# mmdagent/distantspeechrecognition-mirror

Hardware: AMD Instinct MI355X
Metric: decoded_audio_hours_per_sec (higher is better)
Workload: dtype f32

## Files before the change

### distantspeechrecognition-mirror_amd/csrc/k_viterbi.hip

```cpp
#include "common.h"
#include "wfst_graph.h"
#include "lattice.h"
#include "lexicon.h"
#include "wordtrace.h"
#include <algorithm>
#include <cmath>
#include <type_traits>

namespace dsr {

struct Tok { int32_t node; float ac; float lm; uint32_t bp; };
struct TokA { float ac; float lm; uint32_t bp; uint32_t xs; };
struct TokB { int32_t node; int32_t cnt; };
struct XRecD { int32_t dist; float cost; uint32_t meta; float eps1; int32_t dst; int32_t p2; int32_t dstXoff; int32_t dstCnt; };
struct Side { double ttl; float ac; float lm; int32_t rec; uint32_t prevBp; int32_t c; uint32_t next; };
struct CandA { double ttl; float ac; float lm; };
struct CandB { int32_t dst; int32_t next; int32_t rec; uint32_t prevBp; };
struct Bp { uint32_t prev; uint32_t rec; };

static constexpr uint32_t kNone = 0xFFFFFFFFu;
static constexpr uint32_t kEndBit = 0x80000000u;
static constexpr int kThreads = 1024;
static constexpr int kWaves = kThreads / 64;
static constexpr int kFastK = 8;
static constexpr int kB = 2;
static constexpr int kFastC = 24576;
static constexpr int kFastE = 8190;
static constexpr int kP1 = 16;
static constexpr int kW = 4;
static constexpr int kSideLds = 496;

struct GraphDev {
  int nNodes, initial;
  const int* xoff; const XRec* xrec; const XRecD* xrecD; const int* xarc; const int* xpathOff;
  const int* eoff; const ERec* erec; const int* path; const float* pathCost;
  const float* arcCost; const uint32_t* arcOut; const uint32_t* arcIn;
  const int* nodeFinal; const float* nodeCost;
};

struct SegState { int n, status, maxActive, pad; long arenaOff, chunkEnd, arenaUsed; double thresh; long long stat[3]; };

struct DecDev {
  double beam, lmScale, lmPenalty, silPenalty; uint32_t silenceX; int noPen;
  int segFrames, segCount, segQueues, segDrop; long poolCap, poolChunk;    unsigned long long* poolNext; SegState* segState; int* segDone; TokA* saveA; TokB* saveB;
  int maxTok, maxCand; long arenaCap;
  TokA* tokA; TokB* tokB; TokA* ctok; Side* side; int fastOK; int* tokOff; int* tokCnt; int* owner; int* rank; int* chead; CandA* cA; CandB* cB; unsigned* first; unsigned* tags; Bp* arena;
  int* queue; long long* prof;
  int dumpOn; long dumpCap; long* dumpFrameOff; int* dumpNode; float* dumpAc; float* dumpLm; int* dumpArc; long* dumpCount;
  int latOn; long latCap; uint4* lat; double* latTtl; long* latFrameOff; int* arenaLat; int4* latFinal; int* latInfo;
  int topN; TokA* tokA3; TokB* tokB3;
};

struct VitArgs {
  GraphDev G; DecDev D;
  const float* scores; const int* nframesArr; int U, Tmax, nDist;
  dsr_decode_result* res; int* arcsOut; unsigned* wordsOut; int maxPath, useLdsRow, hashN, regionB, cntCap;
};
typedef const __attribute__((address_space(4))) VitArgs* KP;

__device__ __forceinline__ unsigned ld_u32(const unsigned* p) { return __hip_atomic_load(p, __ATOMIC_RELAXED, __HIP_MEMORY_SCOPE_AGENT); }
__device__ __forceinline__ int ld_i32(const int* p) { return __hip_atomic_load(p, __ATOMIC_RELAXED, __HIP_MEMORY_SCOPE_AGENT); }
__device__ __forceinline__ void st_u32(unsigned* p, unsigned v) { __hip_atomic_store(p, v, __ATOMIC_RELAXED, __HIP_MEMORY_SCOPE_AGENT); }
__device__ __forceinline__ void st_i32(int* p, int v) { __hip_atomic_store(p, v, __ATOMIC_RELAXED, __HIP_MEMORY_SCOPE_AGENT); }
__device__ __forceinline__ void st_u64_dev(void* p, unsigned long long v) { __hip_atomic_store(reinterpret_cast<unsigned long long*>(p), v, __ATOMIC_RELAXED, __HIP_MEMORY_SCOPE_AGENT); }
__device__ __forceinline__ unsigned long long ld_u64_dev(const void* p) { return __hip_atomic_load(reinterpret_cast<const unsigned long long*>(p), __ATOMIC_RELAXED, __HIP_MEMORY_SCOPE_AGENT); }

__device__ __forceinline__ int wave_incl_scan(int v, int )
{
  v += __builtin_amdgcn_update_dpp(0, v, 0x111, 0xF, 0xF, true);
  v += __builtin_amdgcn_update_dpp(0, v, 0x112, 0xF, 0xF, true);
  v += __builtin_amdgcn_update_dpp(0, v, 0x114, 0xF, 0xF, true);
  v += __builtin_amdgcn_update_dpp(0, v, 0x118, 0xF, 0xF, true);
  v += __builtin_amdgcn_update_dpp(0, v, 0x142, 0xA, 0xF, false);
  v += __builtin_amdgcn_update_dpp(0, v, 0x143, 0xC, 0xF, false);
  return v;
}
__device__ __forceinline__ float wave_max_f_uni(float v)
{
#define DSR_DPP_F(ctrl, rm) { const float o = __int_as_float(__builtin_amdgcn_update_dpp(__float_as_int(v), __float_as_int(v), ctrl, rm, 0xF, false)); v = fmaxf(v, o); }
  DSR_DPP_F(0x111, 0xF) DSR_DPP_F(0x112, 0xF) DSR_DPP_F(0x114, 0xF) DSR_DPP_F(0x118, 0xF) DSR_DPP_F(0x142, 0xA) DSR_DPP_F(0x143, 0xC)
#undef DSR_DPP_F
  return __int_as_float(__builtin_amdgcn_readlane(__float_as_int(v), 63));
}
__device__ __forceinline__ double wave_min_d_uni(double v)
{
#define DSR_DPP_D(ctrl, rm) { const int lo = __double2loint(v), hi = __double2hiint(v); \
    const double o = __hiloint2double(__builtin_amdgcn_update_dpp(hi, hi, ctrl, rm, 0xF, false), __builtin_amdgcn_update_dpp(lo, lo, ctrl, rm, 0xF, false)); v = (o < v) ? o : v; }
  DSR_DPP_D(0x111, 0xF) DSR_DPP_D(0x112, 0xF) DSR_DPP_D(0x114, 0xF) DSR_DPP_D(0x118, 0xF) DSR_DPP_D(0x142, 0xA) DSR_DPP_D(0x143, 0xC)
#undef DSR_DPP_D
  return __hiloint2double(__builtin_amdgcn_readlane(__double2hiint(v), 63), __builtin_amdgcn_readlane(__double2loint(v), 63));
}
__device__ __forceinline__ double wave_min_d(double v)
{
#pragma unroll
  for (int d = 32; d >= 1; d >>= 1) { const double o = __shfl_xor(v, d, 64); v = (o < v) ? o : v; }
  return v;
}
__device__ __forceinline__ unsigned long long wave_min_u64(unsigned long long v)
{
// ... 27 lines not shown
{
  if (idx < sideLds) {
    const lds_side_t* p = (const lds_side_t*) sideL + idx;
    const unsigned long long a = *reinterpret_cast<const volatile __attribute__((address_space(3))) unsigned long long*>(&p->ac);
    rec = *reinterpret_cast<const volatile __attribute__((address_space(3))) int*>(&p->rec);
    ac = __uint_as_float((unsigned) (a & 0xFFFFFFFFull)); lm = __uint_as_float((unsigned) (a >> 32));
    DSR_NO_MERGE();
  } else {
    const Side* p = side + idx;
    const unsigned long long a = *reinterpret_cast<const volatile unsigned long long*>(&p->ac); rec = *reinterpret_cast<const volatile int*>(&p->rec);
    ac = __uint_as_float((unsigned) (a & 0xFFFFFFFFull)); lm = __uint_as_float((unsigned) (a >> 32));
  }
}
__device__ __forceinline__ void side_link(const Side* sideL, const Side* side, int sideLds, int idx, int& c, double& ttl, unsigned& next)
{
  if (idx < sideLds) { const lds_side_t* p = (const lds_side_t*) sideL + idx; c = p->c; ttl = p->ttl; next = p->next; DSR_NO_MERGE(); }
  else { const Side* p = side + idx; c = p->c; ttl = p->ttl; next = p->next; }
}
__device__ __forceinline__ float side_score(const Side* sideL, const Side* side, int sideLds, int idx)
{
  float r;
  if (idx < sideLds) { const lds_side_t* p = (const lds_side_t*) sideL + idx; r = __fadd_rn(p->ac, p->lm); DSR_NO_MERGE(); }
  else { const Side* p = side + idx; r = __fadd_rn(p->ac, p->lm); }
  return r;
}
template <class T> __device__ __forceinline__ const T* at32(const void* base, uint32_t byteOff) { return reinterpret_cast<const T*>(reinterpret_cast<const char*>(base) + byteOff); }
template <class T> __device__ __forceinline__ T* at32w(void* base, uint32_t byteOff) { return reinterpret_cast<T*>(reinterpret_cast<char*>(base) + byteOff); }
__device__ __forceinline__ int uni(int v) { return __builtin_amdgcn_readfirstlane(v); }
__device__ __forceinline__ double uni(double v) { return __hiloint2double(__builtin_amdgcn_readfirstlane(__double2hiint(v)), __builtin_amdgcn_readfirstlane(__double2loint(v))); }
__device__ __forceinline__ unsigned f2ord(float f) { const unsigned u = __float_as_uint(f); return (u & 0x80000000u) ? ~u : (u | 0x80000000u); }

template <int MODES>
__global__ __launch_bounds__(kThreads) void k_viterbi(const VitArgs argsInKernarg)
{
  (void) argsInKernarg;
  constexpr bool PROF = (MODES & 1) != 0, EXTRA = (MODES & 2) != 0;
  const KP KA = (KP) __builtin_amdgcn_kernarg_segment_ptr();
  KP ka = KA;
#define RELOAD() do { ka = KA; asm volatile("" : "+s"(ka)); } while (0)
  RELOAD();
  extern __shared__ __attribute__((aligned(16))) unsigned char smem[];
  float* srow = reinterpret_cast<float*>(smem);
  const int useLdsRow = ka->useLdsRow, nDist = ka->nDist, hashN = ka->hashN, regionB = ka->regionB, cntCap = ka->cntCap;
  unsigned* hkey = reinterpret_cast<unsigned*>(srow + (useLdsRow ? ((nDist + 3) & ~3) : 4));
  unsigned* hfirst = hkey + hashN;
  Side* sideL = reinterpret_cast<Side*>(hfirst + hashN);
  unsigned short* cntL = reinterpret_cast<unsigned short*>(reinterpret_cast<unsigned char*>(hfirst + hashN) + regionB);
  __shared__ int s_waveTot[kWaves];
  __shared__ int s_waveTotE[kWaves];
  __shared__ double s_waveMin[kWaves];
  __shared__ float s_waveMag[kWaves];
  __shared__ unsigned long long s_waveKey[kWaves];
  __shared__ int s_sideN;
  __shared__ int s_tb[2];
  __shared__ unsigned s_bm[kFastC / 32];
  __shared__ unsigned s_gbase[kFastC / 64 + 4];
  __shared__ int s_cnt[(kFastK + 32) * kWaves];
  __shared__ int s_err;
  __shared__ long long s_prof[32]; __shared__ long long s_tlast;
  __shared__ long long s_stat[3];
  __shared__ int s_maxActive; __shared__ unsigned s_tag; __shared__ long long s_latOff;
  if (PROF && threadIdx.x < 32) s_prof[threadIdx.x] = 0;
#define TICK(ix) do { if (PROF && tid == 0) { const long long tn = (long long) wall_clock64(); s_prof[ix] += tn - s_tlast; s_tlast = tn; } } while (0)
  constexpr int nthr = kThreads, nw = kWaves;
  __shared__ int s_u, s_seg, s_help; __shared__ long long s_chunk;

  const int tid = threadIdx.x;
  const int slot = blockIdx.x;
#define TOKA(ix) ((EXTRA && (ix) == 2) ? ka->D.tokA3 + (size_t) slot * ka->D.maxTok : ka->D.tokA + ((size_t) slot * 2 + (size_t) (ix)) * ka->D.maxTok)
#define TOKB(ix) ((EXTRA && (ix) == 2) ? ka->D.tokB3 + (size_t) slot * ka->D.maxTok : ka->D.tokB + ((size_t) slot * 2 + (size_t) (ix)) * ka->D.maxTok)
#define curA TOKA(bufCur)
#define nxtA TOKA(bufNxt)
#define curB TOKB(bufCur)
#define nxtB TOKB(bufNxt)
#define sprA TOKA(bufSpr)
#define sprB TOKB(bufSpr)
#define ctok (ka->D.ctok + (size_t) slot * 8192)
#define side (ka->D.side + (size_t) slot * kFastC)
#define cA (ka->D.cA + (size_t) slot * ka->D.maxCand)
#define cB (ka->D.cB + (size_t) slot * ka->D.maxCand)
  if (tid == 0) s_tag = ka->D.tags[slot];
#define arena (ka->D.arena + (size_t) ((EXTRA && ka->D.latOn) ? u : (ka->D.segFrames > 0 ? 0 : slot)) * ka->D.arenaCap)
#define sc (ka->scores + (size_t) u * ka->Tmax * nDist)
  constexpr int fastCapC = ((kFastK + 32) * nthr < kFastC) ? (kFastK + 32) * nthr : kFastC;
  constexpr int fastCapN = kP1 * 64 * nw;
  const bool fastOK = ka->D.fastOK && hashN >= 8192;
  const int tableC = (hashN >> 1) + (hashN >> 2), eCap = kFastE, sideLds = regionB >> 5;

  const int nq = (EXTRA || ka->D.segFrames <= 0) ? 1 : ka->D.segQueues;
  const int xcd = nq == 8 ? (int) (__builtin_amdgcn_s_getreg((3 << 11) | 20) & 7u) : 0;
  if (tid == 0) s_help = (nq == 8 && ((ka->D.segDrop >> xcd) & 1)) ? 1 : 0;
  for (;;) {
    __syncthreads();
    if (tid == 0) {
      const int segS0 = EXTRA ? 0 : ka->D.segFrames; int help = s_help, uu = -1, sg = 0;
      for (;;) {
        const int qx = (xcd + help) & (nq - 1), Uq = (ka->U - qx + nq - 1) / nq;
        int it = -1;
        if (help == 0) { it = atomicAdd(ka->D.queue + qx, 1); if (it >= (segS0 > 0 ? ka->D.segCount * Uq : Uq)) it = -1; }
        else {
          int c = ld_i32(ka->D.queue + qx);
          while (c < Uq) { const int prev = atomicCAS(ka->D.queue + qx, c, c + 1); if (prev == c) { it = c; break; } c = prev; }
        }
        if (it >= 0) { uu = segS0 > 0 ? qx + nq * (it % Uq) : it; sg = segS0 > 0 ? it / Uq : 0; break; }
        if (segS0 > 0 && nq == 8 && help < 7) help++; else break;
      }
      if (uu >= 0 && help > 0) { st_i32(&ka->D.segState[uu].status, -2); asm volatile("s_waitcnt vmcnt(0)" ::: "memory"); st_i32(&ka->D.segDone[uu], 0x7FFFFFFF); sg = -1; }
// ... 842 lines not shown
              nxtA[pos] = na; nxtB[pos] = nb; arena[arenaOff + pos] = bp;
              if (EXTRA && ka->D.latOn) ka->D.arenaLat[(size_t) u * ka->D.arenaCap + arenaOff + pos] = (int) (s_latOff + w);
            }
          }
        }
      }
      if (EXTRA && ka->D.latOn) {
        uint4* lat = ka->D.lat + (size_t) u * ka->D.latCap; double* ltt = ka->D.latTtl + (size_t) u * ka->D.latCap;
        const long latOff = (long) s_latOff;
        for (int c = tid; c < C; c += nthr) {
          const CandA a = cA[c]; const CandB b = cB[c];
          lat[latOff + c] = make_uint4(__float_as_uint(a.ac), __float_as_uint(a.lm), (unsigned) b.rec, b.prevBp); ltt[latOff + c] = a.ttl;
        }
        __syncthreads();
        if (tid == 0) { s_latOff = latOff + C; ka->D.latFrameOff[(size_t) u * (ka->Tmax + 3) + fr + 1] = latOff + C; }
      }
      }
      __syncthreads();
      TICK(fast ? 7 : 8);
      RELOAD();
      if (mode == 0) {
        if (dump) {
          long* cnt = ka->D.dumpCount; const long o = cnt[0];
          if (o + numNew <= ka->D.dumpCap) {
            for (int i = tid; i < numNew; i += nthr) {
              const TokA t = ld_tok(&nxtA[i]); ka->D.dumpNode[o + i] = nxtB[i].node; ka->D.dumpAc[o + i] = t.ac; ka->D.dumpLm[o + i] = t.lm;
              ka->D.dumpArc[o + i] = ka->G.xarc[arena[t.bp].rec];
            }
          }
          __syncthreads();
          if (tid == 0) { ka->D.dumpFrameOff[fr] = o; ka->D.dumpFrameOff[fr + 1] = o + numNew; cnt[0] = o + numNew; cnt[1] = fr + 1; }
        }
        if (numStat < 0) numStat = numNew;
        if (numStat == 0 || numNew == 0) { status = DSR_E_CONSISTENCY; break; }
        { const int t = bufCur; bufCur = bufNxt; bufNxt = t; }
        n = numNew; arenaOff += numNew; arenaUsed += numNew;
        if (tid == nthr - 1) { s_stat[0] += numStat; s_stat[1] += Cfr; if (fast) s_stat[2] += 1; if (numStat > s_maxActive) s_maxActive = numStat; }
        thresh = __dadd_rn(topScore, ka->D.beam);
      } else {
        const TokA* lst = numNew > 0 ? nxtA : curA; const int cntL = numNew > 0 ? numNew : n;
        unsigned long long key = ~0ull;
        for (int i = tid; i < cntL; i += nthr) {
          const TokA t = lst[i]; const float s = __fadd_rn(t.ac, t.lm);
          if (s == s) { const unsigned long long k = ((unsigned long long) f2ord(s) << 32) | (unsigned) i; if (k < key) key = k; }
        }
        key = wave_min_u64(key);
        if (lane == 0) s_waveKey[wave] = key;
        if (EXTRA && ka->D.latOn) {
          const TokB* lstB = numNew > 0 ? nxtB : curB; int4* lf = ka->D.latFinal + (size_t) u * ka->D.maxTok;
          for (int i = tid; i < cntL; i += nthr) { const TokA t = ld_tok(&lst[i]); lf[i] = make_int4(lstB[i].node, (int) t.bp, __float_as_int(t.ac), __float_as_int(t.lm)); }
          if (tid == 0) { int* li = ka->D.latInfo + 4 * (size_t) u; li[0] = cntL; li[1] = numNew > 0 ? 1 : 0; li[2] = (int) (arenaOff + (numNew > 0 ? numNew : 0)); li[3] = T; }
        }
        __syncthreads();
        int* hopRec = reinterpret_cast<int*>(cB); const int hopCap = 2 * ka->D.maxCand; int* hopOff = hopRec + hopCap;
        if (tid == 0) {
          dsr_decode_result* const res = ka->res;
          clear_result(&res[u]); dsr_decode_result& r = res[u];
          unsigned long long k = ~0ull; for (int w = 0; w < nw; w++) if (s_waveKey[w] < k) k = s_waveKey[w];
          r.frames = T - 1; r.reachedFinal = numNew > 0 ? 1 : 0; r.finalStatesN = numNew;  r.activeHypos = (long) s_stat[0]; r.placements = (long) s_stat[1] + Cfr; r.registerFrames = (long) s_stat[2]; r.maxActiveSeen = s_maxActive; r.status = DSR_OK;
          int nH = 0;
          if (k != ~0ull) {
            const TokA bt = ld_tok(&lst[(unsigned) (k & 0xFFFFFFFFu)]);
            r.ac = bt.ac; r.lm = bt.lm; r.score = __dadd_rn((double) bt.ac, (double) bt.lm);
            for (uint32_t bq = bt.bp; bq != kNone && nH < hopCap; ) {
              uint2 e; if (segS > 0) { const unsigned long long v = ld_u64_dev(&arena[bq]); e.x = (unsigned) v; e.y = (unsigned) (v >> 32); } else e = *reinterpret_cast<const uint2*>(&arena[bq]);
              hopRec[nH++] = (int) e.y; bq = e.x;
            }
          } else r.status = DSR_E_CONSISTENCY;
          s_tb[0] = nH; s_tb[1] = 0;
        }
        __syncthreads();
        const int nH = s_tb[0];
        auto block_excl = [&](const int v, int& total) -> int {
          const int incl = wave_incl_scan(v, lane);
          if (lane == 63) s_waveTot[wave] = incl;
          __syncthreads();
          int base = 0, tot = 0;
          for (int w = 0; w < nw; w++) { const int q = s_waveTot[w]; if (w < wave) base += q; tot += q; }
          __syncthreads();
          total = tot; return base + incl - v;
        };
        int nA = 0;
        for (int b0 = 0; b0 < nH; b0 += nthr) {
          const int i = b0 + tid; int len = 0;
          if (i < nH) { const uint32_t rc = (uint32_t) hopRec[i]; len = (rc & kEndBit) ? ka->G.erec[rc & ~kEndBit].pathLen : (int) (ka->G.xrec[rc].meta & 0xFFFFu) + 1; }
          int total; const int ex = block_excl(len, total);
          if (i < nH) hopOff[i] = nA + ex;
          nA += total;
        }
        int* const arcsOut = ka->arcsOut; unsigned* const wordsOut = ka->wordsOut; const int maxPath = ka->maxPath; dsr_decode_result* const res = ka->res;
        int* ao = arcsOut ? arcsOut + (size_t) u * maxPath : nullptr;
        int nWloc = 0;
        for (int i = tid; i < nH; i += nthr) {
          const uint32_t rc = (uint32_t) hopRec[i]; int pos = nA - hopOff[i];
          if (rc & kEndBit) {
            const ERec e = ka->G.erec[rc & ~kEndBit];
            for (int h = e.pathLen - 1; h >= 0; h--) { const int a = ka->G.path[e.pathOff + h]; pos--; if (ao && pos < maxPath) ao[pos] = a; if (ka->G.arcOut[a] != 0) nWloc++; }
          } else {
            const int a = ka->G.xarc[rc]; pos--; if (ao && pos < maxPath) ao[pos] = a; if (ka->G.arcOut[a] != 0) nWloc++;
            const int pl = (int) (ka->G.xrec[rc].meta & 0xFFFFu); const int po = ka->G.xpathOff[rc];
            for (int h = pl - 1; h >= 0; h--) { const int a2 = ka->G.path[po + h]; pos--; if (ao && pos < maxPath) ao[pos] = a2; if (ka->G.arcOut[a2] != 0) nWloc++; }
          }
        }
        if (nWloc) atomicAdd(&s_tb[1], nWloc);
        __syncthreads();
        if (wordsOut && ao) {
          unsigned* wo = wordsOut + (size_t) u * maxPath; int q = 0;
          const int lim = nA < maxPath ? nA : maxPath;
          for (int b0 = 0; b0 < lim; b0 += nthr) {
            const int i = b0 + tid; unsigned o = 0u;
            if (i < lim) o = ka->G.arcOut[ao[i]];
            int total; const int ex = block_excl(o != 0u ? 1 : 0, total);
            if (o != 0u && q + ex < maxPath) wo[q + ex] = o;
            q += total;
          }
        }
        if (tid == 0) {
          if (res[u].status == DSR_OK) {
            res[u].nArcs = nA; res[u].nWords = s_tb[1];
            if (nH >= hopCap) res[u].status = DSR_E_ALLOCATION; else if (nA > maxPath && arcsOut) res[u].status = DSR_E_DIMENSION;
          }
        }
        __syncthreads();
        TICK(9);
      }
    }

    RELOAD();
    if (PROF && tid == 0) s_prof[15] = (long long) wall_clock64();
    if (segS > 0 && status == DSR_OK && fr <= T) {
      TokA* const svA = ka->D.saveA + (size_t) u * ka->D.maxTok; TokB* const svB = ka->D.saveB + (size_t) u * ka->D.maxTok;
      for (int i = tid; i < n; i += nthr) { svA[i] = curA[i]; svB[i] = curB[i]; }
      if (tid == 0) {
        SegState* const sst = ka->D.segState + u;
        st_i32(&sst->n, n); st_i32(&sst->status, DSR_OK); st_i32(&sst->maxActive, s_maxActive); st_u64_dev(&sst->arenaOff, (unsigned long long) arenaOff); st_u64_dev(&sst->chunkEnd, (unsigned long long) chunkEnd); st_u64_dev(&sst->arenaUsed, (unsigned long long) arenaUsed);
        st_u64_dev(&sst->thresh, (unsigned long long) __double_as_longlong(thresh));
        st_u64_dev(&sst->stat[0], (unsigned long long) s_stat[0]); st_u64_dev(&sst->stat[1], (unsigned long long) s_stat[1]); st_u64_dev(&sst->stat[2], (unsigned long long) s_stat[2]);
      }
      if (nq == 1) __builtin_amdgcn_fence(__ATOMIC_RELEASE, "agent");
      else __builtin_amdgcn_fence(__ATOMIC_RELEASE, "workgroup");
      __syncthreads();
      if (tid == 0) st_i32(&ka->D.segDone[u], seg + 1);
      continue;
    }
    if (status != DSR_OK) {
      if (tid == 0) {
        dsr_decode_result* const res = ka->res; clear_result(&res[u]); res[u].status = status; res[u].frames = T - 1;
        if (segS > 0) { st_i32(&ka->D.segState[u].status, status); asm volatile("s_waitcnt vmcnt(0)" ::: "memory"); st_i32(&ka->D.segDone[u], 0x7FFFFFFF); }
      }
    }
  }
  RELOAD();
  if (tid == 0) ka->D.tags[slot] = s_tag;
  if (PROF && tid < 32) ka->D.prof[slot * 32 + tid] = s_prof[tid];
#undef TICK
#undef RELOAD
#undef TOKA
#undef TOKB
#undef curA
#undef nxtA
#undef curB
#undef nxtB
#undef sprA
#undef sprB
#undef ctok
#undef side
#undef cA
#undef cB
#undef arena
#undef sc
#undef dump
}

struct DecoderState {
  dsr_decoder_cfg cfg; bool haveGraph = false; int nSlots = 0; int nNodes = 0;
  WfstGraph::Csr csr; WfstGraph::Tables tab;
  DevBuf<int> d_xoff, d_xarc, d_xpathOff, d_eoff, d_path, d_nodeFinal, d_queue; DevBuf<float> d_pathCost;
  DevBuf<XRec> d_xrec; DevBuf<ERec> d_erec; DevBuf<float> d_arcCost, d_nodeCost; DevBuf<uint32_t> d_arcOut, d_arcIn;
  DevBuf<TokA> d_tokA, d_ctok; DevBuf<TokB> d_tokB; DevBuf<Side> d_side; DevBuf<XRecD> d_xrecD; int fastOK = 0; int maxCnt = 0; DevBuf<int> d_tokOff, d_tokCnt, d_owner, d_rank, d_chead; DevBuf<unsigned> d_tags; DevBuf<CandA> d_cA; DevBuf<CandB> d_cB; DevBuf<unsigned> d_first; DevBuf<Bp> d_arena;
  DevBuf<long long> d_prof; DevBuf<dsr_decode_result> d_res; DevBuf<int> d_arcs; DevBuf<unsigned> d_words;
  long arenaCap = 0; int initial = 0; unsigned tokenMemoryLimit = 0;
  long lastPoolCap = 0;
  DevBuf<SegState> d_segState; DevBuf<int> d_segDone; DevBuf<unsigned long long> d_poolNext; DevBuf<TokA> d_saveA; DevBuf<TokB> d_saveB;
  DevBuf<WTok> w_tok; DevBuf<WCand> w_cand; DevBuf<int> w_tokOff, w_rank; DevBuf<unsigned long long> w_best; DevBuf<unsigned> w_first; DevBuf<int4> w_traces; size_t w_tablesFor = 0;
  bool costNegZero = false; double costMinAbs = HUGE_VAL;
  DevBuf<uint4> d_lat; DevBuf<double> d_latTtl; DevBuf<long> d_latFrameOff; DevBuf<int> d_arenaLat; DevBuf<int4> d_latFinal; DevBuf<int> d_latInfo;
  int latU = 0, latTmax = 0; long latArenaCap = 0; WfstGraph graphCopy; DevBuf<TokA> d_tokA3; DevBuf<TokB> d_tokB3;
  const dsr_lexicon* lexIn = nullptr; const dsr_lexicon* lexOut = nullptr; uint32_t eosX = 0; std::string eosSymbol;
  int lastU = 0; size_t lastMaxPath = 0; bool lastPaths = false;
  PinBuf<dsr_decode_result> h_res; PinBuf<int> h_arcs; PinBuf<unsigned> h_words; hipEvent_t evDone = nullptr;
  int pendingU = 0; size_t pendingPath = 0; int pendingSlots = 0; long long* pendingProf = nullptr;
  int dumpOn = 0; long dumpCap = 0; DevBuf<long> d_dumpFrameOff, d_dumpCount; DevBuf<int> d_dumpNode, d_dumpArc; DevBuf<float> d_dumpAc, d_dumpLm;
  std::vector<int64_t> h_dumpFrameOff; std::vector<int32_t> h_dumpNode, h_dumpArc; std::vector<float> h_dumpAc, h_dumpLm; int64_t h_dumpFrames = 0;
};

}

using namespace dsr;
struct dsr_wfst : WfstGraph { dsr_lexicon* lexState = nullptr; dsr_lexicon* lexIn = nullptr; dsr_lexicon* lexOut = nullptr; };
struct dsr_decoder : DecoderState {};

extern "C" {

dsr_status dsr_wfst_create(dsr_wfst** out) { return guard([&] { if (!out) throw Error(DSR_E_PARAMETER, "null argument"); *out = new dsr_wfst(); }); }
dsr_status dsr_wfst_set_sorted_output(dsr_wfst* g, int on)
{ return guard([&] { if (!g) throw Error(DSR_E_PARAMETER, "null argument"); if (!g->arcs.empty()) throw Error(DSR_E_CONSISTENCY, "the transducer already has arcs"); g->sortedOutput = on != 0; }); }
void dsr_wfst_destroy(dsr_wfst* g) { delete g; }
dsr_status dsr_wfst_read(dsr_wfst* g, const char* f, int binary) { return guard([&] { if (!g) throw Error(DSR_E_PARAMETER, "null argument"); g->read(f, binary != 0); }); }
dsr_status dsr_wfst_read_dynamic(dsr_wfst* g, const char* f, int noSelfLoops) { return guard([&] { if (!g) throw Error(DSR_E_PARAMETER, "null argument"); g->readEx(f, false, noSelfLoops != 0); }); }
dsr_status dsr_wfst_write(const dsr_wfst* g, const char* f, int binary) { return guard([&] { if (!g) throw Error(DSR_E_PARAMETER, "null argument"); g->write(f, binary != 0); }); }
dsr_status dsr_wfst_write_symbols(const dsr_wfst* g, const char* f, int binary, int useSymbols)
{ return guard([&] { if (!g) throw Error(DSR_E_PARAMETER, "null argument"); g->write(f, binary != 0, useSymbols != 0); }); }
dsr_status dsr_wfst_reverse(dsr_wfst* g, const dsr_wfst* src)
{ return guard([&] { if (!g || !src) throw Error(DSR_E_PARAMETER, "null argument"); g->reverse(*src); }); }
dsr_status dsr_wfst_reverse_read(dsr_wfst* g, const char* f)
{ return guard([&] { if (!g) throw Error(DSR_E_PARAMETER, "null argument"); g->reverseRead(f); }); }
dsr_status dsr_wfst_add_arc(dsr_wfst* g, unsigned s1, unsigned s2, unsigned in, unsigned out, float cost)
{ return guard([&] { if (!g) throw Error(DSR_E_PARAMETER, "null argument"); g->addArc(s1, s2, in, out, cost, true); }); }
dsr_status dsr_wfst_add_final(dsr_wfst* g, unsigned s, float cost) { return guard([&] { if (!g) throw Error(DSR_E_PARAMETER, "null argument"); g->addFinal(s, cost); }); }
int dsr_wfst_num_nodes(const dsr_wfst* g) { return (int) g->nodes.size(); }
int dsr_wfst_num_arcs(const dsr_wfst* g) { return (int) g->arcs.size(); }
dsr_status dsr_wfst_export(const dsr_wfst* g, uint32_t* nodeState, int32_t* nodeFinal, float* nodeCost, int32_t* arcOff,
                           int32_t* arcDst, uint32_t* arcIn, uint32_t* arcOut, float* arcCost)
{
  return guard([&] {
    if (!g) throw Error(DSR_E_PARAMETER, "null argument");
    const WfstGraph::Csr c = g->csr(); const size_t n = g->nodes.size();
    for (size_t i = 0; i < n; i++) { if (nodeState) nodeState[i] = g->nodes[i].state; if (nodeFinal) nodeFinal[i] = g->nodes[i].final_; if (nodeCost) nodeCost[i] = g->nodes[i].cost; }
    if (arcOff) for (size_t i = 0; i <= n; i++) arcOff[i] = c.off[i];
    for (size_t a = 0; a < c.dst.size(); a++) { if (arcDst) arcDst[a] = c.dst[a]; if (arcIn) arcIn[a] = c.in[a]; if (arcOut) arcOut[a] = c.out[a]; if (arcCost) arcCost[a] = c.cost[a]; }
  });
}
// ... 226 lines not shown
      d->w_tok.reserve(S * 2 * c.maxActive); d->w_cand.reserve(S * c.maxCandidates); d->w_tokOff.reserve(S * (c.maxActive + 1)); d->w_rank.reserve(S * c.maxCandidates);
      d->w_traces.reserve((size_t) U * maxTraces); d->d_queue.reserve(8); d->d_res.reserve(U);
      if (d->w_tablesFor != S * d->nNodes) {
        d->w_best.reserve(S * d->nNodes); d->w_first.reserve(S * d->nNodes); d->w_tablesFor = S * d->nNodes;
        DSR_HIP(hipMemsetAsync(d->w_best.p, 0xFF, sizeof(unsigned long long) * S * d->nNodes, st)); DSR_HIP(hipMemsetAsync(d->w_first.p, 0xFF, sizeof(unsigned) * S * d->nNodes, st));
      }
      if (maxPath < 1) maxPath = 1;
      d->d_arcs.reserve((size_t) U * maxPath); d->d_words.reserve((size_t) U * maxPath);
      DSR_HIP(hipMemsetAsync(d->d_queue.p, 0, 8 * sizeof(int), st));
      WtArgs A; A.nNodes = d->nNodes; A.initial = d->initial; A.xoff = d->d_xoff.p; A.xrec = d->d_xrec.p; A.xarc = d->d_xarc.p; A.xpathOff = d->d_xpathOff.p; A.eoff = d->d_eoff.p;
      A.erec = d->d_erec.p; A.path = d->d_path.p; A.arcCost = d->d_arcCost.p; A.arcOut = d->d_arcOut.p; A.arcIn = d->d_arcIn.p; A.nodeFinal = d->d_nodeFinal.p; A.nodeCost = d->d_nodeCost.p;
      A.beam = c.beam; A.lmScale = c.lmScale; A.lmPenalty = c.lmPenalty; A.silPenalty = c.silPenalty; A.silenceX = c.silenceX; A.insertSilence = c.insertSilence;
      A.maxTok = c.maxActive; A.maxCand = c.maxCandidates; A.maxTraces = maxTraces;
      A.tok = d->w_tok.p; A.cand = d->w_cand.p; A.tokOff = d->w_tokOff.p; A.rank = d->w_rank.p; A.bestKey = d->w_best.p; A.firstSlot = d->w_first.p; A.traces = d->w_traces.p; A.queue = d->d_queue.p;
      A.scores = score; A.nframes = nframes; A.U = U; A.Tmax = Tmax; A.nDist = nDist; A.res = d->d_res.p; A.arcsOut = d->d_arcs.p; A.wordsOut = d->d_words.p; A.maxPath = maxPath;
      wordtrace_launch(A, slots, st);
      const size_t nPath = want_paths ? (size_t) U * maxPath : 0;
      d->h_res.reserve(U); d->h_arcs.reserve(nPath ? nPath : 1); d->h_words.reserve(nPath ? nPath : 1);
      DSR_HIP(hipMemcpyAsync(d->h_res.p, d->d_res.p, sizeof(dsr_decode_result) * U, hipMemcpyDeviceToHost, st));
      if (nPath) DSR_HIP(hipMemcpyAsync(d->h_arcs.p, d->d_arcs.p, sizeof(int) * nPath, hipMemcpyDeviceToHost, st));
      if (nPath) DSR_HIP(hipMemcpyAsync(d->h_words.p, d->d_words.p, sizeof(unsigned) * nPath, hipMemcpyDeviceToHost, st));
      if (!d->evDone) DSR_HIP(hipEventCreateWithFlags(&d->evDone, hipEventDisableTiming));
      DSR_HIP(hipEventRecord(d->evDone, st));
      d->pendingU = U; d->pendingPath = nPath; d->pendingSlots = slots; d->pendingProf = nullptr; d->latU = 0;
      return;
    }
    int32_t* arcs_out = want_paths ? (int32_t*) 1 : nullptr; uint32_t* words_out = want_paths ? (uint32_t*) 1 : nullptr;
    for (size_t a = 0; a < d->csr.in.size(); a++) if (d->csr.in[a] > (uint32_t) nDist) throw Error(DSR_E_INDEX, "arc input %u has no distribution (nDist=%d)", d->csr.in[a], nDist);
    int slots = d->cfg.streams; if (slots > U) slots = U; if (d->dumpOn) slots = 1;
    const bool latOn = d->cfg.latticeTokens > 0;
    if (latOn && d->dumpOn) throw Error(DSR_E_PARAMETER, "lattice bookkeeping and the token dump are separate debugging aids: enable one");
    int segFrames = 0;
    if (!latOn && !d->dumpOn && d->cfg.topN <= 0 && U > slots) {
      segFrames = getenv("DSR_VITERBI_SEG") ? atoi(getenv("DSR_VITERBI_SEG")) : 125;
      if (segFrames < 0 || 2 * segFrames > Tmax + 1) segFrames = 0;
      const double saveGB = (double) U * (double) d->cfg.maxActive * 24.0 / 1e9;
      if (saveGB > (getenv("DSR_VITERBI_SEG_SAVE_GB") ? atof(getenv("DSR_VITERBI_SEG_SAVE_GB")) : 16.0)) segFrames = 0;
    }
    int segQueues = 8;
    if (segFrames > 0 && !(slots >= 64 && slots % 8 == 0 && xcd_round_robin((hipStream_t) stream))) { if (getenv("DSR_VITERBI_SEG_ANY")) segQueues = 1; else segFrames = 0; }
    if (segFrames > 0 && getenv("DSR_VITERBI_SEG_ANY") && atoi(getenv("DSR_VITERBI_SEG_ANY")) == 2) segQueues = 1;
    const long arenaPer = d->cfg.arenaTokens > 0 ? (long) d->cfg.arenaTokens : (long) 8192 * (long) (Tmax + 2);
    int poolArenas = 0;
    if (segFrames > 0) {
      const double want = (double) U * 1536.0 * (double) (Tmax + 2) / (double) arenaPer;
      poolArenas = (int) std::min<double>(std::ceil(want), (double) (0xFFFFFFF0u / (unsigned long long) arenaPer));
      if ((unsigned long long) std::max(poolArenas, slots) * (unsigned long long) arenaPer > 0xFFFFFFF0ull) segFrames = 0;
    }
    ensure_scratch(d, slots, Tmax, latOn ? U : (segFrames > 0 ? poolArenas : 0));
    d->d_res.reserve(U);
    if (maxPath < 0) maxPath = 0;
    if (arcs_out || words_out) { d->d_arcs.reserve((size_t) U * (maxPath > 0 ? maxPath : 1)); d->d_words.reserve((size_t) U * (maxPath > 0 ? maxPath : 1)); }
    DSR_HIP(hipMemsetAsync(d->d_queue.p, 0, 8 * sizeof(int), st));
    if (d->dumpOn) {
      d->dumpCap = (long) d->cfg.maxActive * 64 < (long) 1 << 26 ? (long) 1 << 24 : (long) 1 << 26;
      d->d_dumpFrameOff.reserve(Tmax + 2); d->d_dumpCount.reserve(2);
      d->d_dumpNode.reserve(d->dumpCap); d->d_dumpArc.reserve(d->dumpCap); d->d_dumpAc.reserve(d->dumpCap); d->d_dumpLm.reserve(d->dumpCap);
      DSR_HIP(hipMemsetAsync(d->d_dumpCount.p, 0, 2 * sizeof(long), st));
    }
    GraphDev G; G.nNodes = d->nNodes; G.initial = d->initial; G.xoff = d->d_xoff.p; G.xrec = d->d_xrec.p; G.xrecD = d->d_xrecD.p; G.xarc = d->d_xarc.p;
    G.xpathOff = d->d_xpathOff.p; G.eoff = d->d_eoff.p; G.erec = d->d_erec.p; G.path = d->d_path.p; G.pathCost = d->d_pathCost.p; G.arcCost = d->d_arcCost.p;
    G.arcOut = d->d_arcOut.p; G.arcIn = d->d_arcIn.p; G.nodeFinal = d->d_nodeFinal.p; G.nodeCost = d->d_nodeCost.p;
    DecDev D; D.beam = d->cfg.beam; D.lmScale = d->cfg.lmScale; D.lmPenalty = d->cfg.lmPenalty; D.silPenalty = d->cfg.silPenalty;
    D.noPen = (d->cfg.lmScale > 0.0 && std::isfinite(d->cfg.lmScale) && d->cfg.lmScale * d->cfg.lmPenalty == 0.0 && d->cfg.lmScale * d->cfg.silPenalty == 0.0 &&
               !d->costNegZero && (d->costMinAbs == HUGE_VAL || d->cfg.lmScale * d->costMinAbs >= 0x1p-60) && !getenv("DSR_VITERBI_PEN")) ? 1 : 0;
    D.silenceX = d->cfg.silenceX; D.maxTok = d->cfg.maxActive; D.maxCand = d->cfg.maxCandidates; D.arenaCap = d->arenaCap;
    D.tokA = d->d_tokA.p; D.tokB = d->d_tokB.p; D.ctok = d->d_ctok.p; D.side = d->d_side.p; D.fastOK = d->fastOK; D.tokOff = d->d_tokOff.p; D.owner = d->d_owner.p; D.rank = d->d_rank.p; D.cA = d->d_cA.p; D.cB = d->d_cB.p;
    D.first = d->d_first.p; D.tags = d->d_tags.p; D.tokCnt = d->d_tokCnt.p; D.chead = d->d_chead.p; D.arena = d->d_arena.p; D.queue = d->d_queue.p;
    if (getenv("DSR_VITERBI_SEG_VERBOSE")) fprintf(stderr, "[dsr viterbi] %d utterances on %d workgroups: %s\n", U, slots, segFrames > 0 ? (segQueues == 8 ? "time-sliced, XCD-bound queues" : "time-sliced, one queue") : "run to completion");
    D.segDrop = getenv("DSR_VITERBI_SEG_DROP") ? (int) strtol(getenv("DSR_VITERBI_SEG_DROP"), nullptr, 0) : 0;
    D.segQueues = segQueues; D.segFrames = segFrames; D.segCount = segFrames > 0 ? (Tmax + segFrames) / segFrames : 1;
    D.poolCap = 0; D.poolChunk = 0; D.poolNext = nullptr; D.segState = nullptr; D.segDone = nullptr; D.saveA = nullptr; D.saveB = nullptr;
    if (segFrames > 0) {
      d->d_segState.reserve(U); d->d_segDone.reserve(U); d->d_poolNext.reserve(1);
      d->d_saveA.reserve((size_t) U * d->cfg.maxActive); d->d_saveB.reserve((size_t) U * d->cfg.maxActive);
      DSR_HIP(hipMemsetAsync(d->d_segDone.p, 0, sizeof(int) * (size_t) U, st)); DSR_HIP(hipMemsetAsync(d->d_poolNext.p, 0, sizeof(unsigned long long), st));
      D.poolCap = (long) ((size_t) std::max(poolArenas, slots) * (size_t) d->arenaCap); if (D.poolCap > (long) 0xFFFFFFF0L) D.poolCap = (long) 0xFFFFFFF0L;
      D.poolChunk = std::min<long>(262144, std::max<long>(4096, D.poolCap / (4 * (long) U)));
      D.poolNext = d->d_poolNext.p; D.segState = d->d_segState.p; D.segDone = d->d_segDone.p; D.saveA = d->d_saveA.p; D.saveB = d->d_saveB.p;
    }
    d->lastPoolCap = D.poolCap;
    D.prof = nullptr;
    if (getenv("DSR_VITERBI_PROF")) { d->d_prof.reserve((size_t) slots * 32); D.prof = d->d_prof.p; }
    D.dumpOn = d->dumpOn; D.dumpCap = d->dumpCap; D.dumpFrameOff = d->d_dumpFrameOff.p; D.dumpNode = d->d_dumpNode.p; D.dumpAc = d->d_dumpAc.p;
    D.dumpLm = d->d_dumpLm.p; D.dumpArc = d->d_dumpArc.p; D.dumpCount = d->d_dumpCount.p;
    D.topN = d->cfg.topN > 0 ? d->cfg.topN : 0; D.tokA3 = nullptr; D.tokB3 = nullptr;
    if (D.topN > 0) { d->d_tokA3.reserve((size_t) slots * d->cfg.maxActive); d->d_tokB3.reserve((size_t) slots * d->cfg.maxActive); D.tokA3 = d->d_tokA3.p; D.tokB3 = d->d_tokB3.p; }
    D.latOn = latOn ? 1 : 0; D.latCap = 0; D.lat = nullptr; D.latTtl = nullptr; D.latFrameOff = nullptr; D.arenaLat = nullptr; D.latFinal = nullptr; D.latInfo = nullptr;
    if (latOn) {
      const size_t cap = (size_t) d->cfg.latticeTokens;
      d->d_lat.reserve((size_t) U * cap); d->d_latTtl.reserve((size_t) U * cap); d->d_latFrameOff.reserve((size_t) U * (Tmax + 3));
      d->d_arenaLat.reserve((size_t) U * (size_t) d->arenaCap); d->d_latFinal.reserve((size_t) U * d->cfg.maxActive); d->d_latInfo.reserve((size_t) 4 * U);
      DSR_HIP(hipMemsetAsync(d->d_latInfo.p, 0, sizeof(int) * 4 * (size_t) U, st));
      D.latCap = (long) cap; D.lat = d->d_lat.p; D.latTtl = d->d_latTtl.p; D.latFrameOff = d->d_latFrameOff.p; D.arenaLat = d->d_arenaLat.p; D.latFinal = d->d_latFinal.p; D.latInfo = d->d_latInfo.p;
      d->latU = U; d->latTmax = Tmax; d->latArenaCap = d->arenaCap;
    } else d->latU = 0;
    const int modes = (D.prof ? 1 : 0) | ((latOn || D.topN > 0 || d->dumpOn) ? 2 : 0);
    const void* kfn = modes == 0 ? (const void*) k_viterbi<0> : modes == 1 ? (const void*) k_viterbi<1> : modes == 2 ? (const void*) k_viterbi<2> : (const void*) k_viterbi<3>;
    hipFuncAttributes fattr; DSR_HIP(hipFuncGetAttributes(&fattr, kfn));
    const size_t eoffB = (size_t) kSideLds * sizeof(Side); const size_t ldsCap = (size_t) 160 * 1024 - fattr.sharedSizeBytes;
    const int hashMax = 16384;
    int useLds = (size_t) nDist * sizeof(float) <= 64 * 1024;
    if (useLds && (size_t) ((nDist + 3) & ~3) * sizeof(float) + (size_t) hashMax * 8 + eoffB > ldsCap) useLds = 0;
    const size_t rowB = useLds ? (size_t) ((nDist + 3) & ~3) * sizeof(float) : 16;
    int hashN = hashMax; while (hashN > 0 && rowB + (size_t) hashN * 8 + eoffB > ldsCap) hashN >>= 1;
    if (getenv("DSR_VITERBI_NOHASH")) hashN = 0;
    int cntCap = (hashN > 0 && d->maxCnt < 65536 && rowB + (size_t) hashN * 8 + eoffB + 4096 <= ldsCap) ? 2048 : 0;
    if (getenv("DSR_VITERBI_NOCNT")) cntCap = 0;
    const size_t lds = rowB + (size_t) hashN * 8 + eoffB + 2 * (size_t) cntCap;
    VitArgs A; A.G = G; A.D = D; A.scores = score; A.nframesArr = nframes; A.U = U; A.Tmax = Tmax; A.nDist = nDist; A.res = d->d_res.p;
    A.arcsOut = (arcs_out || words_out) ? d->d_arcs.p : nullptr; A.wordsOut = (arcs_out || words_out) ? d->d_words.p : nullptr; A.maxPath = maxPath;
    A.useLdsRow = useLds; A.hashN = hashN; A.regionB = (int) eoffB; A.cntCap = cntCap;
#define DSR_LAUNCH_V(MM) { DSR_HIP(hipFuncSetAttribute((const void*) k_viterbi<MM>, hipFuncAttributeMaxDynamicSharedMemorySize, (int) lds)); \
      hipLaunchKernelGGL(k_viterbi<MM>, dim3(slots), dim3(kThreads), lds, st, A); }
    switch (modes) { case 0: DSR_LAUNCH_V(0) break; case 1: DSR_LAUNCH_V(1) break; case 2: DSR_LAUNCH_V(2) break; default: DSR_LAUNCH_V(3) break; }
#undef DSR_LAUNCH_V
    DSR_HIP(hipGetLastError());
    const size_t nPath = want_paths ? (size_t) U * maxPath : 0;
    d->h_res.reserve(U); d->h_arcs.reserve(nPath ? nPath : 1); d->h_words.reserve(nPath ? nPath : 1);
    DSR_HIP(hipMemcpyAsync(d->h_res.p, d->d_res.p, sizeof(dsr_decode_result) * U, hipMemcpyDeviceToHost, st));
    if (nPath) DSR_HIP(hipMemcpyAsync(d->h_arcs.p, d->d_arcs.p, sizeof(int) * nPath, hipMemcpyDeviceToHost, st));
    if (nPath) DSR_HIP(hipMemcpyAsync(d->h_words.p, d->d_words.p, sizeof(unsigned) * nPath, hipMemcpyDeviceToHost, st));
    if (!d->evDone) DSR_HIP(hipEventCreateWithFlags(&d->evDone, hipEventDisableTiming));
    DSR_HIP(hipEventRecord(d->evDone, st));
    d->pendingU = U; d->pendingPath = nPath; d->pendingSlots = slots; d->pendingProf = D.prof;
  });
}

dsr_status dsr_decoder_decode_collect(dsr_decoder* d, dsr_decode_result* res, int32_t* arcs_out, uint32_t* words_out)
{
  return guard([&] {
    if (!d || !res) throw Error(DSR_E_PARAMETER, "null argument");
    if (d->pendingU <= 0) throw Error(DSR_E_CONSISTENCY, "no decode in flight");
    const int U = d->pendingU; const size_t nPath = d->pendingPath; const int slots = d->pendingSlots; long long* prof = d->pendingProf;
    d->pendingU = 0; d->lastU = U; d->lastPaths = nPath > 0; d->lastMaxPath = nPath > 0 ? nPath / (size_t) U : 0;
    DSR_HIP(hipEventSynchronize(d->evDone));
    memcpy(res, d->h_res.p, sizeof(dsr_decode_result) * U);
    if (arcs_out && nPath) memcpy(arcs_out, d->h_arcs.p, sizeof(int) * nPath);
    if (words_out && nPath) memcpy(words_out, d->h_words.p, sizeof(unsigned) * nPath);
    if (getenv("DSR_VITERBI_SEG_VERBOSE") && d->d_poolNext.p && d->lastPoolCap > 0) {
      unsigned long long used = 0; DSR_HIP(hipMemcpy(&used, d->d_poolNext.p, sizeof(used), hipMemcpyDeviceToHost));
      fprintf(stderr, "[dsr viterbi] pool of back-pointer records: %.1f M of %.1f M taken\n", used / 1e6, d->lastPoolCap / 1e6);
    }
    if (prof) {
      std::vector<long long> hp((size_t) slots * 32); DSR_HIP(hipMemcpy(hp.data(), prof, hp.size() * sizeof(long long), hipMemcpyDeviceToHost));
      double acc[32] = {0}; for (int s2 = 0; s2 < slots; s2++) for (int i = 0; i < 32; i++) acc[i] += (double) hp[(size_t) s2 * 32 + i];
      fprintf(stderr, "[dsr viterbi prof] mean us per slot:");
      for (int i = 0; i < 32; i++) if (i != 15) fprintf(stderr, " p%d=%.0f", i, acc[i] / slots / 100.0);
      fprintf(stderr, "\n");
      double tmin = 1e30, tmax = 0.0, tsum = 0.0;
      for (int s2 = 0; s2 < slots; s2++) { double t = 0.0; for (int i = 0; i < 32; i++) if (i != 15) t += (double) hp[(size_t) s2 * 32 + i]; t /= 100.0; tsum += t; if (t < tmin) tmin = t; if (t > tmax) tmax = t; }
      fprintf(stderr, "[dsr viterbi prof] busy us per slot: mean %.0f min %.0f max %.0f\n", tsum / slots, tmin, tmax);
      if (slots >= 64 && slots % 8 == 0) {
        double bx[8] = {0}; for (int s2 = 0; s2 < slots; s2++) { double t = 0.0; for (int i = 0; i < 32; i++) if (i != 15) t += (double) hp[(size_t) s2 * 32 + i]; bx[s2 & 7] += t / 100.0; }
        fprintf(stderr, "[dsr viterbi prof] busy us per slot, by XCD:"); for (int q = 0; q < 8; q++) fprintf(stderr, " %.0f", bx[q] / (slots / 8)); fprintf(stderr, "\n");
      }
    }
    if (d->dumpOn) {
      long cnt[2]; DSR_HIP(hipMemcpy(cnt, d->d_dumpCount.p, sizeof(cnt), hipMemcpyDeviceToHost));
      const long N = cnt[0] < d->dumpCap ? cnt[0] : d->dumpCap; d->h_dumpFrames = cnt[1];
      std::vector<long> fo(cnt[1] + 1); if (cnt[1] > 0) DSR_HIP(hipMemcpy(fo.data(), d->d_dumpFrameOff.p, sizeof(long) * (cnt[1] + 1), hipMemcpyDeviceToHost));
      d->h_dumpFrameOff.assign(fo.begin(), fo.end());
      d->h_dumpNode.resize(N); d->h_dumpArc.resize(N); d->h_dumpAc.resize(N); d->h_dumpLm.resize(N);
      if (N > 0) {
        DSR_HIP(hipMemcpy(d->h_dumpNode.data(), d->d_dumpNode.p, sizeof(int) * N, hipMemcpyDeviceToHost));
        DSR_HIP(hipMemcpy(d->h_dumpArc.data(), d->d_dumpArc.p, sizeof(int) * N, hipMemcpyDeviceToHost));
        DSR_HIP(hipMemcpy(d->h_dumpAc.data(), d->d_dumpAc.p, sizeof(float) * N, hipMemcpyDeviceToHost));
        DSR_HIP(hipMemcpy(d->h_dumpLm.data(), d->d_dumpLm.p, sizeof(float) * N, hipMemcpyDeviceToHost));
      }
    }
// ... 129 lines not shown
```

Measured before the change: 23.46.

## Move per-utterance traceback out of Viterbi kernel into separate kernel

The backpointer walk and arc/word emission that ran at the end of each utterance inside the 1024-thread Viterbi workgroup are moved to a new k_traceback kernel with one 256-thread block per utterance. The Viterbi kernel now only records the best token's backpointer (and, in the simple case, the hop list) into a small per-utterance info buffer. This frees the large decoding workgroup from serial traceback work and block-wide scans, so it can move on to the next utterance sooner. The cost is an extra kernel launch, extra global buffers, and a serial single-thread arena walk in the new kernel for pooled or lattice modes. That walk relies on the arena still being valid after the main kernel finishes.

```diff
diff --git a/distantspeechrecognition-mirror_amd/csrc/k_viterbi.hip b/distantspeechrecognition-mirror_amd/csrc/k_viterbi.hip
--- a/distantspeechrecognition-mirror_amd/csrc/k_viterbi.hip
+++ b/distantspeechrecognition-mirror_amd/csrc/k_viterbi.hip
@@ -45,6 +45,7 @@
   int segFrames, segCount, segQueues, segDrop; long poolCap, poolChunk;    unsigned long long* poolNext; SegState* segState; int* segDone; TokA* saveA; TokB* saveB;
   int maxTok, maxCand; long arenaCap;
   TokA* tokA; TokB* tokB; TokA* ctok; Side* side; int fastOK; int* tokOff; int* tokCnt; int* owner; int* rank; int* chead; CandA* cA; CandB* cB; unsigned* first; unsigned* tags; Bp* arena;
+  int4* tbInfo; int* tbHops; int tbWalkCap;
   int* queue; long long* prof;
   int dumpOn; long dumpCap; long* dumpFrameOff; int* dumpNode; float* dumpAc; float* dumpLm; int* dumpArc; long* dumpCount;
   int latOn; long latCap; uint4* lat; double* latTtl; long* latFrameOff; int* arenaLat; int4* latFinal; int* latInfo;
@@ -178,7 +179,6 @@
   __shared__ float s_waveMag[kWaves];
   __shared__ unsigned long long s_waveKey[kWaves];
   __shared__ int s_sideN;
-  __shared__ int s_tb[2];
   __shared__ unsigned s_bm[kFastC / 32];
   __shared__ unsigned s_gbase[kFastC / 64 + 4];
   __shared__ int s_cnt[(kFastK + 32) * kWaves];
@@ -1127,77 +1127,25 @@
           if (tid == 0) { int* li = ka->D.latInfo + 4 * (size_t) u; li[0] = cntL; li[1] = numNew > 0 ? 1 : 0; li[2] = (int) (arenaOff + (numNew > 0 ? numNew : 0)); li[3] = T; }
         }
         __syncthreads();
-        int* hopRec = reinterpret_cast<int*>(cB); const int hopCap = 2 * ka->D.maxCand; int* hopOff = hopRec + hopCap;
         if (tid == 0) {
           dsr_decode_result* const res = ka->res;
           clear_result(&res[u]); dsr_decode_result& r = res[u];
           unsigned long long k = ~0ull; for (int w = 0; w < nw; w++) if (s_waveKey[w] < k) k = s_waveKey[w];
           r.frames = T - 1; r.reachedFinal = numNew > 0 ? 1 : 0; r.finalStatesN = numNew;  r.activeHypos = (long) s_stat[0]; r.placements = (long) s_stat[1] + Cfr; r.registerFrames = (long) s_stat[2]; r.maxActiveSeen = s_maxActive; r.status = DSR_OK;
-          int nH = 0;
           if (k != ~0ull) {
             const TokA bt = ld_tok(&lst[(unsigned) (k & 0xFFFFFFFFu)]);
             r.ac = bt.ac; r.lm = bt.lm; r.score = __dadd_rn((double) bt.ac, (double) bt.lm);
-            for (uint32_t bq = bt.bp; bq != kNone && nH < hopCap; ) {
-              uint2 e; if (segS > 0) { const unsigned long long v = ld_u64_dev(&arena[bq]); e.x = (unsigned) v; e.y = (unsigned) (v >> 32); } else e = *reinterpret_cast<const uint2*>(&arena[bq]);
-              hopRec[nH++] = (int) e.y; bq = e.x;
-            }
+            const bool perUtt = EXTRA && ka->D.latOn, pool = ka->D.segFrames > 0;
+            const int aix = perUtt ? u : (pool ? 0 : slot);
+            int nH = -1;
+            if (!perUtt && !pool) {
+              const int walkCap = ka->D.tbWalkCap; int* const hopRec = ka->D.tbHops + (size_t) u * 2 * walkCap; nH = 0;
+              for (uint32_t bq = bt.bp; bq != kNone && nH < walkCap; ) { const uint2 e = *reinterpret_cast<const uint2*>(&arena[bq]); hopRec[nH++] = (int) e.y; bq = e.x; }
+            }
+            ka->D.tbInfo[u] = make_int4(nH < 0 ? 1 : 2, (int) bt.bp, aix, nH);
           } else r.status = DSR_E_CONSISTENCY;
-          s_tb[0] = nH; s_tb[1] = 0;
         }
         __syncthreads();
-        const int nH = s_tb[0];
-        auto block_excl = [&](const int v, int& total) -> int {
-          const int incl = wave_incl_scan(v, lane);
-          if (lane == 63) s_waveTot[wave] = incl;
-          __syncthreads();
-          int base = 0, tot = 0;
-          for (int w = 0; w < nw; w++) { const int q = s_waveTot[w]; if (w < wave) base += q; tot += q; }
-          __syncthreads();
-          total = tot; return base + incl - v;
-        };
-        int nA = 0;
-        for (int b0 = 0; b0 < nH; b0 += nthr) {
-          const int i = b0 + tid; int len = 0;
-          if (i < nH) { const uint32_t rc = (uint32_t) hopRec[i]; len = (rc & kEndBit) ? ka->G.erec[rc & ~kEndBit].pathLen : (int) (ka->G.xrec[rc].meta & 0xFFFFu) + 1; }
-          int total; const int ex = block_excl(len, total);
-          if (i < nH) hopOff[i] = nA + ex;
-          nA += total;
-        }
-        int* const arcsOut = ka->arcsOut; unsigned* const wordsOut = ka->wordsOut; const int maxPath = ka->maxPath; dsr_decode_result* const res = ka->res;
-        int* ao = arcsOut ? arcsOut + (size_t) u * maxPath : nullptr;
-        int nWloc = 0;
-        for (int i = tid; i < nH; i += nthr) {
-          const uint32_t rc = (uint32_t) hopRec[i]; int pos = nA - hopOff[i];
-          if (rc & kEndBit) {
-            const ERec e = ka->G.erec[rc & ~kEndBit];
-            for (int h = e.pathLen - 1; h >= 0; h--) { const int a = ka->G.path[e.pathOff + h]; pos--; if (ao && pos < maxPath) ao[pos] = a; if (ka->G.arcOut[a] != 0) nWloc++; }
-          } else {
-            const int a = ka->G.xarc[rc]; pos--; if (ao && pos < maxPath) ao[pos] = a; if (ka->G.arcOut[a] != 0) nWloc++;
-            const int pl = (int) (ka->G.xrec[rc].meta & 0xFFFFu); const int po = ka->G.xpathOff[rc];
-            for (int h = pl - 1; h >= 0; h--) { const int a2 = ka->G.path[po + h]; pos--; if (ao && pos < maxPath) ao[pos] = a2; if (ka->G.arcOut[a2] != 0) nWloc++; }
-          }
-        }
-        if (nWloc) atomicAdd(&s_tb[1], nWloc);
-        __syncthreads();
-        if (wordsOut && ao) {
-          unsigned* wo = wordsOut + (size_t) u * maxPath; int q = 0;
-          const int lim = nA < maxPath ? nA : maxPath;
-          for (int b0 = 0; b0 < lim; b0 += nthr) {
-            const int i = b0 + tid; unsigned o = 0u;
-            if (i < lim) o = ka->G.arcOut[ao[i]];
-            int total; const int ex = block_excl(o != 0u ? 1 : 0, total);
-            if (o != 0u && q + ex < maxPath) wo[q + ex] = o;
-            q += total;
-          }
-        }
-        if (tid == 0) {
-          if (res[u].status == DSR_OK) {
-            res[u].nArcs = nA; res[u].nWords = s_tb[1];
-            if (nH >= hopCap) res[u].status = DSR_E_ALLOCATION; else if (nA > maxPath && arcsOut) res[u].status = DSR_E_DIMENSION;
-          }
-        }
-        __syncthreads();
-        TICK(9);
       }
     }
 
@@ -1247,12 +1195,89 @@
 #undef dump
 }
 
+static constexpr int kTbThreads = 256;
+struct TbArgs {
+  const XRec* xrec; const ERec* erec; const int* xarc; const int* xpathOff; const int* path; const uint32_t* arcOut;
+  const Bp* arena; long arenaCap; const int4* tbInfo;
+  int* hops;
+  int walkCap;
+  dsr_decode_result* res; int* arcsOut; unsigned* wordsOut; int maxPath;
+};
+__global__ __launch_bounds__(kTbThreads) void k_traceback(const TbArgs a)
+{
+  constexpr int nthr = kTbThreads, nw = kTbThreads / 64;
+  __shared__ int s_waveTot[nw]; __shared__ int s_tb[2];
+  const int u = blockIdx.x, tid = threadIdx.x, lane = tid & 63, wave = tid >> 6;
+  const int4 info = a.tbInfo[u];
+  if (info.x == 0) return;
+  int* const hopRec = a.hops + (size_t) u * 2 * a.walkCap; int* const hopOff = hopRec + a.walkCap;
+  if (tid == 0) {
+    int nH = info.w;
+    if (info.x == 1) {
+      const Bp* const arena = a.arena + (size_t) info.z * a.arenaCap; nH = 0;
+      for (uint32_t bq = (uint32_t) info.y; bq != kNone && nH < a.walkCap; ) { const uint2 e = *reinterpret_cast<const uint2*>(&arena[bq]); hopRec[nH++] = (int) e.y; bq = e.x; }
+    }
+    s_tb[0] = nH; s_tb[1] = 0;
+  }
+  __syncthreads();
+  const int nH = s_tb[0];
+  auto block_excl = [&](const int v, int& total) -> int {
+    const int incl = wave_incl_scan(v, lane);
+    if (lane == 63) s_waveTot[wave] = incl;
+    __syncthreads();
+    int base = 0, tot = 0;
+    for (int w = 0; w < nw; w++) { const int q = s_waveTot[w]; if (w < wave) base += q; tot += q; }
+    __syncthreads();
+    total = tot; return base + incl - v;
+  };
+  int nA = 0;
+  for (int b0 = 0; b0 < nH; b0 += nthr) {
+    const int i = b0 + tid; int len = 0;
+    if (i < nH) { const uint32_t rc = (uint32_t) hopRec[i]; len = (rc & kEndBit) ? a.erec[rc & ~kEndBit].pathLen : (int) (a.xrec[rc].meta & 0xFFFFu) + 1; }
+    int total; const int ex = block_excl(len, total);
+    if (i < nH) hopOff[i] = nA + ex;
+    nA += total;
+  }
+  const int maxPath = a.maxPath;
+  int* ao = a.arcsOut ? a.arcsOut + (size_t) u * maxPath : nullptr;
+  int nWloc = 0;
+  for (int i = tid; i < nH; i += nthr) {
+    const uint32_t rc = (uint32_t) hopRec[i]; int pos = nA - hopOff[i];
+    if (rc & kEndBit) {
+      const ERec e = a.erec[rc & ~kEndBit];
+      for (int h = e.pathLen - 1; h >= 0; h--) { const int ar = a.path[e.pathOff + h]; pos--; if (ao && pos < maxPath) ao[pos] = ar; if (a.arcOut[ar] != 0) nWloc++; }
+    } else {
+      const int ar = a.xarc[rc]; pos--; if (ao && pos < maxPath) ao[pos] = ar; if (a.arcOut[ar] != 0) nWloc++;
+      const int pl = (int) (a.xrec[rc].meta & 0xFFFFu); const int po = a.xpathOff[rc];
+      for (int h = pl - 1; h >= 0; h--) { const int a2 = a.path[po + h]; pos--; if (ao && pos < maxPath) ao[pos] = a2; if (a.arcOut[a2] != 0) nWloc++; }
+    }
+  }
+  if (nWloc) atomicAdd(&s_tb[1], nWloc);
+  __syncthreads();
+  if (a.wordsOut && ao) {
+    unsigned* wo = a.wordsOut + (size_t) u * maxPath; int q = 0;
+    const int lim = nA < maxPath ? nA : maxPath;
+    for (int b0 = 0; b0 < lim; b0 += nthr) {
+      const int i = b0 + tid; unsigned o = 0u;
+      if (i < lim) o = a.arcOut[ao[i]];
+      int total; const int ex = block_excl(o != 0u ? 1 : 0, total);
+      if (o != 0u && q + ex < maxPath) wo[q + ex] = o;
+      q += total;
+    }
+  }
+  if (tid == 0) {
+    a.res[u].nArcs = nA; a.res[u].nWords = s_tb[1];
+    if (nH >= a.walkCap) a.res[u].status = DSR_E_ALLOCATION; else if (nA > maxPath && a.arcsOut) a.res[u].status = DSR_E_DIMENSION;
+  }
+}
+
 struct DecoderState {
   dsr_decoder_cfg cfg; bool haveGraph = false; int nSlots = 0; int nNodes = 0;
   WfstGraph::Csr csr; WfstGraph::Tables tab;
   DevBuf<int> d_xoff, d_xarc, d_xpathOff, d_eoff, d_path, d_nodeFinal, d_queue; DevBuf<float> d_pathCost;
   DevBuf<XRec> d_xrec; DevBuf<ERec> d_erec; DevBuf<float> d_arcCost, d_nodeCost; DevBuf<uint32_t> d_arcOut, d_arcIn;
   DevBuf<TokA> d_tokA, d_ctok; DevBuf<TokB> d_tokB; DevBuf<Side> d_side; DevBuf<XRecD> d_xrecD; int fastOK = 0; int maxCnt = 0; DevBuf<int> d_tokOff, d_tokCnt, d_owner, d_rank, d_chead; DevBuf<unsigned> d_tags; DevBuf<CandA> d_cA; DevBuf<CandB> d_cB; DevBuf<unsigned> d_first; DevBuf<Bp> d_arena;
+  DevBuf<int4> d_tbInfo; DevBuf<int> d_tbHops;
   DevBuf<long long> d_prof; DevBuf<dsr_decode_result> d_res; DevBuf<int> d_arcs; DevBuf<unsigned> d_words;
   long arenaCap = 0; int initial = 0; unsigned tokenMemoryLimit = 0;
   long lastPoolCap = 0;
@@ -1585,6 +1610,8 @@
     if (maxPath < 0) maxPath = 0;
     if (arcs_out || words_out) { d->d_arcs.reserve((size_t) U * (maxPath > 0 ? maxPath : 1)); d->d_words.reserve((size_t) U * (maxPath > 0 ? maxPath : 1)); }
     DSR_HIP(hipMemsetAsync(d->d_queue.p, 0, 8 * sizeof(int), st));
+    const int walkCap = (int) std::min<long>(2L * d->cfg.maxCandidates, (long) Tmax + 2);
+    d->d_tbInfo.reserve(U); d->d_tbHops.reserve((size_t) U * 2 * (size_t) walkCap); DSR_HIP(hipMemsetAsync(d->d_tbInfo.p, 0, sizeof(int4) * (size_t) U, st));
     if (d->dumpOn) {
       d->dumpCap = (long) d->cfg.maxActive * 64 < (long) 1 << 26 ? (long) 1 << 24 : (long) 1 << 26;
       d->d_dumpFrameOff.reserve(Tmax + 2); d->d_dumpCount.reserve(2);
@@ -1599,7 +1626,7 @@
                !d->costNegZero && (d->costMinAbs == HUGE_VAL || d->cfg.lmScale * d->costMinAbs >= 0x1p-60) && !getenv("DSR_VITERBI_PEN")) ? 1 : 0;
     D.silenceX = d->cfg.silenceX; D.maxTok = d->cfg.maxActive; D.maxCand = d->cfg.maxCandidates; D.arenaCap = d->arenaCap;
     D.tokA = d->d_tokA.p; D.tokB = d->d_tokB.p; D.ctok = d->d_ctok.p; D.side = d->d_side.p; D.fastOK = d->fastOK; D.tokOff = d->d_tokOff.p; D.owner = d->d_owner.p; D.rank = d->d_rank.p; D.cA = d->d_cA.p; D.cB = d->d_cB.p;
-    D.first = d->d_first.p; D.tags = d->d_tags.p; D.tokCnt = d->d_tokCnt.p; D.chead = d->d_chead.p; D.arena = d->d_arena.p; D.queue = d->d_queue.p;
+    D.first = d->d_first.p; D.tags = d->d_tags.p; D.tokCnt = d->d_tokCnt.p; D.chead = d->d_chead.p; D.arena = d->d_arena.p; D.queue = d->d_queue.p; D.tbInfo = d->d_tbInfo.p; D.tbHops = d->d_tbHops.p; D.tbWalkCap = walkCap;
     if (getenv("DSR_VITERBI_SEG_VERBOSE")) fprintf(stderr, "[dsr viterbi] %d utterances on %d workgroups: %s\n", U, slots, segFrames > 0 ? (segQueues == 8 ? "time-sliced, XCD-bound queues" : "time-sliced, one queue") : "run to completion");
     D.segDrop = getenv("DSR_VITERBI_SEG_DROP") ? (int) strtol(getenv("DSR_VITERBI_SEG_DROP"), nullptr, 0) : 0;
     D.segQueues = segQueues; D.segFrames = segFrames; D.segCount = segFrames > 0 ? (Tmax + segFrames) / segFrames : 1;
@@ -1649,6 +1676,13 @@
     switch (modes) { case 0: DSR_LAUNCH_V(0) break; case 1: DSR_LAUNCH_V(1) break; case 2: DSR_LAUNCH_V(2) break; default: DSR_LAUNCH_V(3) break; }
 #undef DSR_LAUNCH_V
     DSR_HIP(hipGetLastError());
+    {
+      TbArgs B; B.xrec = G.xrec; B.erec = G.erec; B.xarc = G.xarc; B.xpathOff = G.xpathOff; B.path = G.path; B.arcOut = G.arcOut;
+      B.arena = D.arena; B.arenaCap = D.arenaCap; B.tbInfo = D.tbInfo; B.hops = d->d_tbHops.p; B.walkCap = walkCap;
+      B.res = A.res; B.arcsOut = A.arcsOut; B.wordsOut = A.wordsOut; B.maxPath = A.maxPath;
+      hipLaunchKernelGGL(k_traceback, dim3(U), dim3(kTbThreads), 0, st, B);
+      DSR_HIP(hipGetLastError());
+    }
     const size_t nPath = want_paths ? (size_t) U * maxPath : 0;
     d->h_res.reserve(U); d->h_arcs.reserve(nPath ? nPath : 1); d->h_words.reserve(nPath ? nPath : 1);
     DSR_HIP(hipMemcpyAsync(d->h_res.p, d->d_res.p, sizeof(dsr_decode_result) * U, hipMemcpyDeviceToHost, st));
```

Result: no change. 23.58 (median of 6 runs) (+0.5%).
